# EternalEvan/InstaRevive

Hardware: AMD Instinct MI355X
Metric: 512->2048 one-step SR images/sec (higher is better)
Workload: dtype bf16; 1 GPU; 512x512 LQ, sr_scale 4 -> 2048x2048 network input, untiled, batch 1 per GPU, full SwinIR->VAE-enc->DiT(t=400)->VAE-dec path; global_batch=1, parallelism=dp1, weights=seeded random, full-size architectures

## Files before the change

### include/instarevive_hip.h

```cpp
#ifndef INSTAREVIVE_HIP_H
#define INSTAREVIVE_HIP_H
#include <stddef.h>
#include <stdint.h>
#ifdef __cplusplus
extern "C" {
#endif

typedef struct ir_ctx ir_ctx;

enum { IR_STAGE_SWINIR = 0, IR_STAGE_VAE_ENCODE = 1, IR_STAGE_DIT = 2, IR_STAGE_VAE_DECODE = 3, IR_STAGE_PIPELINE = 4,
       IR_STAGE_COLORFIX = 5, IR_STAGE_T5 = 6 ,
       IR_STAGE_CLDM = 7 , IR_STAGE_CLDM_PIPELINE = 8 ,
       IR_STAGE_CLIP_TEXT = 9 ,
       IR_STAGE_PNG = 10 ,
       IR_STAGE_RESAMPLE = 11 ,
       IR_STAGE_METRICS = 12 ,
       IR_STAGE_LPIPS = 13 ,
       IR_STAGE_NIQE = 14 ,
       IR_STAGE_CLIPIQA = 15 ,
       IR_STAGE_DEGRADE = 16  };
enum { IR_FLAG_NO_PREPROCESS = 1, IR_FLAG_TILED = 2, IR_FLAG_FIX_WAVELET = 4, IR_FLAG_FIX_ADAIN = 8,
       IR_FLAG_CONTROL_LQ = 16,
       IR_FLAG_GRAPH = 32,
       IR_FLAG_FP8 = 64 };
// ... 169 lines not shown
int ir_op_geglu(ir_ctx* ctx, void* stream, const uint16_t* ag, uint16_t* out, long rows, int f);

int ir_op_attention_d512_fp8(ir_ctx* ctx, void* stream, const uint16_t* q, const uint16_t* k, const uint16_t* v, uint16_t* o, int b, int t, float scale,
                             void* ws, size_t ws_bytes);
int ir_op_attention_fp8(ir_ctx* ctx, void* stream, const uint16_t* q, const uint16_t* k, const uint16_t* v, uint16_t* o, int b, int heads, int t,
                        float scale, void* ws, size_t ws_bytes);
int ir_op_swin_attention(ir_ctx* ctx, void* stream, const uint16_t* qkv, uint16_t* out, const float* bias_t, int b, int h, int w,
                         int heads, int shift, float scale);
int ir_op_swin_mlp(ir_ctx* ctx, void* stream, const float* x, float* out, uint16_t* out2, const void* w_tiles, const float* vec, long t, int c,
                   int hid_p, float eps, const float* next_g, const float* next_b, const void* qkv_tiles, const float* qkv_b, int qkv_n);
int ir_op_swin_attn_proj(ir_ctx* ctx, void* stream, const uint16_t* qkv, const float* xres, float* out, const void* proj_t, const float* proj_b,
                         const float* bias_t, int b, int h, int w, int shift, float scale);
int ir_op_swin_block(ir_ctx* ctx, void* stream, const uint16_t* qkv, const float* x_in, float* x_out, uint16_t* out2, const void* proj_t,
                     const float* proj_b, const float* bias_t, int b, int h, int w, int shift, float scale, const void* w_tiles, const float* vec,
                     int c, int hid_p, float eps, const float* next_g, const float* next_b, const void* qkv_tiles, const float* qkv_b, int qkv_n);
int ir_op_softmax_rows(ir_ctx* ctx, void* stream, const float* x, uint16_t* y, int rows, int cols);
int ir_op_nchw_to_nhwc(ir_ctx* ctx, void* stream, const float* in, uint16_t* out, int n, int ch, long hw, int cpad, float scale, float shift);
int ir_op_nhwc_to_nchw(ir_ctx* ctx, void* stream, const float* in, int in_cs, float* out, int n, int ch, long hw, float scale, float shift, int clamp01);

#ifdef __cplusplus
}
#endif
#endif
```

### instarevive_amd/_lib.py

```python
import ctypes as C
import os

import torch

_HERE = os.path.dirname(os.path.abspath(__file__))
LIB_PATH = os.environ.get("INSTAREVIVE_HIP_LIB") or os.path.join(_HERE, "csrc", "libinstarevive_hip.so")

SYMBOLS = [
    "ir_abi_version", "ir_init", "ir_destroy", "ir_last_error", "ir_upload", "ir_drop_optional", "ir_has_tensor",
    "ir_swinir_configure", "ir_vae_configure", "ir_dit_configure", "ir_dit_control_configure", "ir_dit_set_prompt", "ir_t5_configure", "ir_t5_encode", "ir_workspace_bytes",
    "ir_swinir_forward", "ir_vae_encode", "ir_dit_forward", "ir_dit_step", "ir_dit_forward_control", "ir_dit_step_control", "ir_vae_decode", "ir_color_fix",
    "ir_pipeline", "ir_u8_to_nchw", "ir_nchw_to_u8", "ir_profile_begin", "ir_profile_select", "ir_profile_end", "ir_profile_end_kernels", "ir_profile_kernel_count",
    "ir_profile_kernel_name",
    "ir_op_conv", "ir_op_conv_splitk", "ir_op_conv_groupnorm", "ir_op_linear", "ir_op_groupnorm", "ir_op_layernorm", "ir_op_attention", "ir_op_swin_attention",
    "ir_op_swin_mlp", "ir_op_swin_attn_proj", "ir_op_swin_block", "ir_op_dit_block", "ir_op_softmax_rows", "ir_op_nchw_to_nhwc", "ir_op_nhwc_to_nchw",
    "ir_tiled_count", "ir_tiled_encode", "ir_tiled_encode_part", "ir_tiled_encode_overflow", "ir_op_conv_up2x2", "ir_op_conv_norm", "ir_op_vae_conv_in", "ir_op_vae_norm_conv_out", "ir_op_conv64", "ir_op_conv64_to3", "ir_tiled_dit", "ir_tiled_blend_latent", "ir_tiled_decode", "ir_tiled_blend_pixels", "ir_set_plain_kernels", "ir_set_fp8", "ir_set_fp8_mask", "ir_attn_fallback_count", "ir_op_conv_fp8", "ir_op_conv_fp8_up", "ir_op_conv_fp8_route", "ir_fp8_features", "ir_op_attention_fp8", "ir_op_attention_d512_fp8",
    "ir_unet_configure", "ir_unet_set_context", "ir_cldm_sample", "ir_cldm_pipeline", "ir_clip_text_configure", "ir_clip_text_encode", "ir_op_groupnorm_any", "ir_op_geglu",
    "ir_dit_set_prompts", "ir_op_attention_kv_groups", "ir_graph_records", "ir_op_vae_segment", "ir_op_vae_segment_ws", "ir_op_vae_segment_info",
    "ir_png_bound", "ir_png_encode", "ir_resample_plan_bytes", "ir_resample_plan", "ir_resample_u8", "ir_metrics_y",
    "ir_lpips_scale_table", "ir_lpips_configure", "ir_lpips", "ir_niqe_window", "ir_niqe_stats",
    "ir_clipiqa_scale_table", "ir_clipiqa_configure", "ir_clipiqa", "ir_degrade_qtables", "ir_degrade",
]

STAGE_SWINIR, STAGE_VAE_ENCODE, STAGE_DIT, STAGE_VAE_DECODE, STAGE_PIPELINE, STAGE_COLORFIX, STAGE_T5, STAGE_CLDM, STAGE_CLDM_PIPELINE, STAGE_CLIP_TEXT, STAGE_PNG, STAGE_RESAMPLE, STAGE_METRICS = range(13)
STAGE_LPIPS = 13
STAGE_NIQE = 14
STAGE_CLIPIQA = 15
STAGE_DEGRADE = 16
DEGRADE_NORM_NONE, DEGRADE_NORM_MAX = 0, 1
DEGRADE_MAX_KSIZE, DEGRADE_MIN_LOW = 41, 8
# ... 62 lines not shown
    lib.ir_profile_kernel_name.argtypes = [i]
    lib.ir_profile_kernel_name.restype = C.c_char_p
    lib.ir_u8_to_nchw.argtypes = [vp, vp, vp, vp, i, i, i]
    lib.ir_nchw_to_u8.argtypes = [vp, vp, vp, vp, i, i, i]
    lib.ir_op_conv.argtypes = [vp, vp, vp, vp, vp, vp, i, i, i, i, i, i, i, i, i, i, i, f, vp, i, i]
    lib.ir_op_conv_splitk.argtypes = [vp, vp, vp, vp, vp, vp, i, i, i, i, i, i, i, vp, i, i, vp, sz, C.POINTER(C.c_int)]
    lib.ir_op_conv_groupnorm.argtypes = [vp, vp, vp, vp, vp, vp, vp, vp, vp, i, i, i, i, i, i, i, vp, i, vp, sz, C.POINTER(C.c_int)]
    lib.ir_op_linear.argtypes = [vp, vp, vp, vp, vp, vp, i, i, i, i, i, vp, vp, i, i, f]
    lib.ir_op_groupnorm.argtypes = [vp, vp, vp, vp, vp, vp, i, i, i, i, f, i, vp, sz]
    lib.ir_op_layernorm.argtypes = [vp, vp, vp, vp, vp, vp, i, i, i, i, f]
    lib.ir_op_attention.argtypes = [vp, vp, vp, vp, vp, vp, i, i, i, i, i, f, vp, vp, sz]
    lib.ir_op_swin_attention.argtypes = [vp, vp, vp, vp, vp, i, i, i, i, i, f]
    lib.ir_op_swin_mlp.argtypes = [vp, vp, vp, vp, vp, vp, vp, C.c_long, i, i, f, vp, vp, vp, vp, i]
    lib.ir_op_swin_attn_proj.argtypes = [vp, vp, vp, vp, vp, vp, vp, vp, i, i, i, i, f]
    lib.ir_op_swin_block.argtypes = [vp, vp, vp, vp, vp, vp, vp, vp, vp, i, i, i, i, f, vp, vp, i, i, f, vp, vp, vp, vp, i]
    lib.ir_op_dit_block.argtypes = [vp, vp, vp, i, i, i, i, f, vp, sz]
    lib.ir_op_softmax_rows.argtypes = [vp, vp, vp, vp, i, i]
    lib.ir_op_nchw_to_nhwc.argtypes = [vp, vp, vp, vp, i, i, C.c_long, i, f, f]
    lib.ir_op_nhwc_to_nchw.argtypes = [vp, vp, vp, i, vp, i, i, C.c_long, f, f, i]
    lib.ir_tiled_count.argtypes = [i, i, i, i]
    lib.ir_tiled_encode.argtypes = [vp, vp, vp, vp, vp, vp, i, i, i, i, f, vp, sz]
    lib.ir_tiled_encode_part.argtypes = [vp, vp, vp, vp, vp, vp, i, i, i, i, f, i, i, i, vp, vp, vp, sz]
    lib.ir_tiled_encode_overflow.argtypes = [vp, vp]
    lib.ir_op_conv_up2x2.argtypes = [vp, vp, vp, vp, vp, vp, i, i, i, i, i]
    lib.ir_op_conv_norm.argtypes = [vp, vp, vp, vp, vp, vp, vp, vp, vp, i, i, i, i, i]
    lib.ir_op_vae_conv_in.argtypes = [vp, vp, vp, vp, vp, vp, vp, i, i, i, f, f, vp]
    lib.ir_op_vae_norm_conv_out.argtypes = [vp, vp, vp, vp, vp, vp, vp, vp, i, i, i]
    lib.ir_op_conv64.argtypes = [vp, vp, vp, vp, vp, vp, i, i, i, i, f]
    lib.ir_op_conv64_to3.argtypes = [vp, vp, vp, vp, vp, vp, i, i, i]
    lib.ir_tiled_dit.argtypes = [vp, vp, vp, vp, i, i, i, i, i, i, i, f, f, i, vp, sz]
# ... 152 lines not shown
```

### instarevive_amd/csrc/api.cpp

```cpp
#include <hip/hip_runtime.h>
#include <math.h>
#include <stdarg.h>
#include <stdio.h>
#include <string.h>

#include <algorithm>
#include <memory>
#include <string>
#include <unordered_map>
#include <vector>

#include "../../include/instarevive_hip.h"
#include "kernels.h"

enum { ACT_NONE = 0, ACT_GELU_ERF = 1, ACT_GELU_TANH = 2, ACT_LRELU = 3, ACT_SILU = 4 };

namespace {

struct Tensor {
    void* p = nullptr;
    size_t bytes = 0;
};

struct Conv {
// ... 539 lines not shown
    float* xa = r.a.alloc<float>(T * Cp);
    float* xb = r.a.alloc<float>(T * Cp);
    bf16_t* xn = r.a.alloc<bf16_t>(T * Cp);
    bf16_t* qkv = r.a.alloc<bf16_t>(T * 3 * m.heads * 32);
    bf16_t* att = r.a.alloc<bf16_t>(T * Cp);
    bf16_t* hid = r.a.alloc<bf16_t>(T * m.hid_p);
    bf16_t* xc = r.a.alloc<bf16_t>(T * Cp);
    LAUNCH(r, PC_OTHER, 0.0, 0.0, ir_launch_swin_prep(in, f0, n, h, w, m.mean, m.range, r.s), "swin_prep");
    conv(r, m.conv_first, f0, n, gh, gw, 192, x0, Cp, 1, 1, 1, 0, ACT_NONE, 0.f, nullptr, 0, 0);
    layernorm(r, x0, nullptr, xa, m.pe.g, m.pe.b, T, m.C, Cp, Cp, 1e-5f);
    const float scale = 1.0f / sqrtf((float)m.C / (float)m.heads);
    for (const SwinLayer& L : m.layers) {
        const float* cur = xa;
        bool have_ln1 = false;
        bool have_qkv = false;
        for (size_t j = 0; j < L.blocks.size(); ++j) {
            const SwinBlock& b = L.blocks[j];
            const bool last = j + 1 == L.blocks.size();
            if (!have_qkv) {
                if (!have_ln1) layernorm(r, cur, xn, nullptr, b.n1.g, b.n1.b, T, m.C, Cp, Cp, 1e-5f);
                linear(r, b.qkv, xn, (int)T, Cp, qkv, 3 * m.heads * 32, 0, ACT_NONE, nullptr, 0, 0);
            }
            have_ln1 = have_qkv = false;
            const bool fuse_ln = !last && (m.C & 3) == 0;
            const SwinBlock* nb = fuse_ln ? &L.blocks[j + 1] : nullptr;
            const bool fuse_qkv = nb && nb->qkv_t && nb->qkv.b;
            const double f_attn = 4.0 * (double)T * 64 * m.C + 2.0 * (double)T * m.C * m.C;
            const double f_mlp = 4.0 * (double)T * m.C * m.hid + (fuse_qkv ? 6.0 * (double)T * m.C * m.C : 0.0);
            const double b_mlp = 4.0 * (double)T * m.C * 2 + (fuse_qkv ? 2.0 * (double)T * 3 * m.C : 0.0);
            bf16_t* mlp_out2 = last ? xc : (fuse_qkv ? qkv : (fuse_ln ? xn : nullptr));
            const int shift = (j & 1) ? 4 : 0;
            const float* fbias = shift ? b.biasM : b.biasT;
            const bool fused_attn = b.proj_t && fbias && !g_ir_plain_kernels && (long)T * 576 * 2 < (1L << 32);
            if (fused_attn && b.mlp_t) {
                LAUNCHK(r, PK_SWIN_BLOCK, f_attn + f_mlp, b_mlp + 2.0 * (double)T * 3 * m.C,
                       ir_launch_swin_block(qkv, cur, xb, mlp_out2, b.proj_t, b.proj.b, fbias, n, gh, gw, shift, scale, b.mlp_t, b.mlp_v, m.C, m.hid_p,
                                            1e-5f, r.s, nb ? nb->n1.g : nullptr, nb ? nb->n1.b : nullptr, fuse_qkv ? nb->qkv_t : nullptr,
                                            fuse_qkv ? nb->qkv.b : nullptr, fuse_qkv ? 3 * m.heads * 32 : 0), "swin_block");
                have_ln1 = fuse_ln && !fuse_qkv;
// ... 3164 lines not shown
}
int ir_op_swin_attn_proj(ir_ctx* c, void* stream, const uint16_t* qkv, const float* xres, float* out, const void* proj_t, const float* proj_b,
                         const float* bias_t, int b, int h, int w, int shift, float scale) {
    use_ctx(c);
    int rc = ir_launch_swin_attn_proj(qkv, xres, out, proj_t, proj_b, bias_t, b, h, w, shift, scale, (hipStream_t)stream);
    return rc ? fail(c, rc, "swin_attn_proj failed (%d)", rc) : 0;
}
int ir_op_swin_block(ir_ctx* c, void* stream, const uint16_t* qkv, const float* x_in, float* x_out, uint16_t* out2, const void* proj_t,
                     const float* proj_b, const float* bias_t, int b, int h, int w, int shift, float scale, const void* w_tiles, const float* vec,
                     int ch, int hid_p, float eps, const float* next_g, const float* next_b, const void* qkv_tiles, const float* qkv_b, int qkv_n) {
    use_ctx(c);
    int rc = ir_launch_swin_block(qkv, x_in, x_out, out2, proj_t, proj_b, bias_t, b, h, w, shift, scale, w_tiles, vec, ch, hid_p, eps,
                                  (hipStream_t)stream, next_g, next_b, qkv_tiles, qkv_b, qkv_n);
    return rc ? fail(c, rc, "swin_block failed (%d)", rc) : 0;
}
int ir_op_nchw_to_nhwc(ir_ctx* c, void* stream, const float* in, uint16_t* out, int n, int ch, long hw, int cpad, float scale, float shift) {
    use_ctx(c);
    int rc = ir_launch_nchw_to_nhwc_bf16(in, out, n, ch, hw, cpad, scale, shift, (hipStream_t)stream);
    return rc ? fail(c, rc, "nchw_to_nhwc failed (%d)", rc) : 0;
}
int ir_op_nhwc_to_nchw(ir_ctx* c, void* stream, const float* in, int in_cs, float* out, int n, int ch, long hw, float scale, float shift, int clamp01) {
    use_ctx(c);
    int rc = ir_launch_nhwc_to_nchw(in, in_cs, out, n, ch, hw, scale, shift, clamp01, (hipStream_t)stream);
    return rc ? fail(c, rc, "nhwc_to_nchw failed (%d)", rc) : 0;
}
int ir_op_groupnorm_any(ir_ctx* c, void* stream, const uint16_t* x, uint16_t* y, const float* gamma, const float* beta, int n, long hw, int ch,
                        int groups, float eps, int silu, void* ws, size_t ws_bytes) {
    if (!c || !x || !y || !ws) return fail(c, -1, "ir_op_groupnorm_any: null argument");
    if (ws_bytes < (size_t)ir_gn_any_ws_floats(n, hw, ch) * 4) return fail(c, -20, "ir_op_groupnorm_any: workspace too small");
    use_ctx(c);
// ... 17 lines not shown
```

### instarevive_amd/csrc/kernels.h

```cpp
#pragma once
#include <hip/hip_runtime.h>
#include <stdint.h>

typedef uint16_t bf16_t;

extern int g_ir_plain_kernels;

struct IGemmParams {
    const bf16_t* in;
    int NB, H, W;
    int Cin;
    int in_cs;
    int Ho, Wo;
    int taps;
    int stride;
    int pad;
    int up;
    const bf16_t* wgt;
    long wgt_rs;
    int Cout, Cout_pad, M;
    const float* bias;
    int act;
    float slope;
    float out_scale;
// ... 96 lines not shown
int ir_launch_swin_attn(const bf16_t* qkv, bf16_t* out, const float* biasT, int B, int H, int W, int heads, int ld, int ldo,
                        int shift, float scale, hipStream_t s);
int ir_launch_softmax_rows(const float* x, bf16_t* y, long rows, int cols, long ldx, long ldy, hipStream_t s);
static inline int ir_attn_dv(int D) { return (D + 31) & ~31; }

int ir_launch_swin_mlp(const float* x, float* out, bf16_t* out2, const void* w_tiles, const float* vec, long T, int C, int hid_p, float eps,
                       hipStream_t s, const float* next_g = nullptr, const float* next_b = nullptr, const void* qkv_tiles = nullptr,
                       const float* qkv_b = nullptr, int qkv_n = 0);
int ir_launch_swin_attn_proj(const bf16_t* qkv, const float* xres, float* out, const void* proj_t, const float* proj_b, const float* biasT, int B,
                             int H, int W, int shift, float scale, hipStream_t s);

int ir_launch_swin_block(const bf16_t* qkv, const float* x_in, float* x_out, bf16_t* out2, const void* proj_t, const float* proj_b, const float* biasT,
                         int B, int H, int W, int shift, float scale, const void* w_tiles, const float* vec, int C, int hid_p, float eps, hipStream_t s,
                         const float* next_g = nullptr, const float* next_b = nullptr, const void* qkv_tiles = nullptr, const float* qkv_b = nullptr,
                         int qkv_n = 0);

int ir_launch_t5_embed(const int* ids, const bf16_t* table, float* x, long rows, int D, int vocab, int* bad, hipStream_t s);
int ir_launch_t5_rmsnorm(const float* x, const float* w, bf16_t* yb, float* yf, long rows, int D, float eps, hipStream_t s);
int ir_launch_t5_attn(const bf16_t* qkv, const float* bias, const float* key_mask, bf16_t* out, int B, int T, int H, int dk, hipStream_t s);
int ir_launch_t5_gated_gelu(const bf16_t* ab, bf16_t* out, long rows, int F, hipStream_t s);

#ifndef IR_PNG_ROWS
#define IR_PNG_ROWS 8
#endif
#define IR_PNG_HEADER_BITS 1106
int ir_launch_png_encode(const uint8_t* img, int n, int h, long pitch, int vh, int vw, uint8_t* out, size_t out_stride, uint32_t* info,
                         uint32_t* hist, uint32_t* codes, uint32_t* header, uint32_t* chunk_bytes, uint8_t* slots, long slot_cap, hipStream_t s);

#define IR_RESAMPLE_MAGIC 0x52535038
#define IR_RESAMPLE_HEADER 16
// ... 107 lines not shown
```

### instarevive_amd/csrc/swin_fused.hip

```cpp
#include "common.h"
#include "kernels.h"

typedef __attribute__((address_space(3))) void* sw_lds_t;
IR_DEVINL void sw_glds16(const void* g, sw_lds_t l) { __builtin_amdgcn_global_load_lds(g, l, 16, 0, 0); }

namespace swf {
constexpr int CP = 192;
constexpr int W1_ROW = 400, W1_TILE = 13312;
constexpr int W2_ROW = 80, W2_TILE = 15360;
constexpr int SLOT = W1_TILE + W2_TILE;
constexpr int PIECES = SLOT / 1024;
constexpr int VEC_OFF = 2 * SLOT;
constexpr int NEXT_OFF = 1152;
constexpr int STG_OFF = VEC_OFF + 6144;
constexpr int STG_WAVE = 3 * 4096;
constexpr int LDS_TOTAL = STG_OFF + 8 * STG_WAVE;
}

template <bool LN_NEXT, bool QKV = false>
__global__ __launch_bounds__(512, 1) void swin_mlp_kernel(const float* __restrict__ x, float* __restrict__ out, bf16_t* __restrict__ out2,
                                                          const unsigned char* __restrict__ w, const float* __restrict__ vec, long T, int C,
                                                          int NJ, float eps, const float* __restrict__ next_g, const float* __restrict__ next_b,
                                                          const unsigned char* __restrict__ wq, const float* __restrict__ bq, int NQ) {
    using namespace swf;
// ... 415 lines not shown
    }
}

int ir_launch_swin_attn_proj(const bf16_t* qkv, const float* xres, float* out, const void* proj_t, const float* proj_b, const float* biasT, int B,
                             int H, int W, int shift, float scale, hipStream_t s) {
    if (H <= 0 || W <= 0 || (H & 7) || (W & 7) || shift < 0 || shift >= 8 || B <= 0) return -2;
    if ((long)B * H * W * 576 * 2 >= (1L << 32)) return -4;
    const long n_waves = 2L * B * (H >> 3) * (W >> 3);
    const long blocks = (n_waves + 3) / 4;
    if (blocks > 0x7fffffffL) return -4;
    hipLaunchKernelGGL(swin_attn_proj_kernel, dim3((unsigned)blocks), dim3(256), 0, s, qkv, xres, out, reinterpret_cast<const bf16_t*>(proj_t), proj_b, biasT, H, W,
                       shift, scale * 1.44269504088896340736f, n_waves);
    return hipGetLastError() == hipSuccess ? 0 : -1;
}

template <bool LN_NEXT, bool QKV>
__global__ __launch_bounds__(512, 1) void swin_block_kernel(const bf16_t* __restrict__ qkv, const float* __restrict__ x_in, float* __restrict__ x_out,
                                                            bf16_t* __restrict__ out2, const bf16_t* __restrict__ proj_t,
                                                            const float* __restrict__ proj_b, const float* __restrict__ biasT, int H, int W, int shift,
                                                            float scale_log2, long n_waves, const unsigned char* __restrict__ w,
                                                            const float* __restrict__ vec, int C, int NJ, float eps, const float* __restrict__ next_g,
                                                            const float* __restrict__ next_b, const unsigned char* __restrict__ wq,
                                                            const float* __restrict__ bq, int NQ) {
    using namespace swf;
    constexpr int HEADS = 6, LD = 3 * CP;
#ifdef IR_SWIN_STAMPS
    unsigned long long stp[8];
    stp[0] = __builtin_amdgcn_s_memrealtime();
#define IR_STAMP(k) stp[k] = __builtin_amdgcn_s_memrealtime()
#else
#define IR_STAMP(k)
#endif
    extern __shared__ __attribute__((aligned(1024))) unsigned char smem[];
    const int tid = threadIdx.x, lane = tid & 63, wid = tid >> 6;
    const int wu = __builtin_amdgcn_readfirstlane(wid);
    const int r = lane & 31, h = lane >> 5;
    long wv = (long)blockIdx.x * 8 + wu;
    const bool active = wv < n_waves;
    if (!active) wv = n_waves - 1;

    const int NS = NJ + (QKV ? NQ / 2 : 0);
    auto stage = [&](int jt, int slot) {
        const unsigned char* src = (QKV && jt >= NJ ? wq + (long)(jt - NJ) * SLOT : w + (long)jt * SLOT) + lane * 16;
#pragma unroll
        for (int i = 0; i < 4; ++i)
            if (wu + 8 * i < PIECES) sw_glds16(src + (wu + 8 * i) * 1024, (sw_lds_t)(smem + slot * SLOT + (wu + 8 * i) * 1024));
    };
    stage(0, 0);
    float* vs = reinterpret_cast<float*>(smem + VEC_OFF);
    const int nvec = 3 * CP + 32 * NJ;
    for (int i = tid; i < nvec; i += 512) vs[i] = vec[i];
    constexpr bool ln_next = LN_NEXT;
    if (ln_next)
        for (int i = tid; i < 2 * CP; i += 512) {
            const int c = i < CP ? i : i - CP;
            vs[NEXT_OFF + i] = c < C ? (i < CP ? next_g[c] : next_b[c]) : 0.f;
        }

    const int g = (int)(wv & 1);
    long wlin = wv >> 1;
    const int nwx = W >> 3, nwy = H >> 3;
    const int wx = (int)(wlin % nwx); wlin /= nwx;
    const int wy = (int)(wlin % nwy);
    const long img = wlin / nwy;
    auto tok = [&](int i) {
        int y = wy * 8 + (i >> 3) + shift, x = wx * 8 + (i & 7) + shift;
        if (y >= H) y -= H;
        if (x >= W) x -= W;
        return (long)y * W + x;
    };
    const long tbase = img * H * W;
    const long qtok = tbase + tok(32 * g + r);
    f32x16 yacc[6];
    {
        const long ktok[2] = {tbase + tok(r), tbase + tok(32 + r)};
        const int cls = shift ? ((wy == nwy - 1 ? 2 : 0) | (wx == nwx - 1 ? 1 : 0)) : 0;
        bf16x8 idf[2];
#pragma unroll
        for (int ks = 0; ks < 2; ++ks) {
            uint32_t w4[4];
#pragma unroll
            for (int e2 = 0; e2 < 4; ++e2) {
                const int c0 = 16 * ks + 8 * h + 2 * e2;
                w4[e2] = (c0 == r ? 0x3f80u : 0u) | (c0 + 1 == r ? 0x3f800000u : 0u);
            }
            idf[ks] = __builtin_bit_cast(bf16x8, make_uint4(w4[0], w4[1], w4[2], w4[3]));
        }
#pragma unroll
        for (int ct = 0; ct < 6; ++ct)
// ... 61 lines not shown
                    o = mfma32(__builtin_bit_cast(bf16x8, swa_pack8(vt, 8 * s2, 1.0f)), __builtin_bit_cast(bf16x8, swa_pack8_valu(s[kt], 8 * s2, 1.0f)), o);
            }
            const float inv = 1.0f / rs;
            const bf16x8 ob[2] = {__builtin_bit_cast(bf16x8, swa_pack8_valu(o, 0, inv)), __builtin_bit_cast(bf16x8, swa_pack8_valu(o, 8, inv))};
#pragma unroll
            for (int ct = 0; ct < 6; ++ct)
#pragma unroll
                for (int s2 = 0; s2 < 2; ++s2) {
                    const bf16x8 wp = *reinterpret_cast<const bf16x8*>(proj_t + (((hd * 6 + ct) * 2 + s2) * 64 + lane) * 8);
                    yacc[ct] = mfma32(wp, ob[s2], yacc[ct]);
                }
        }
    }

    IR_STAMP(1);
    unsigned char* stg = smem + STG_OFF + wu * STG_WAVE;
    const int ptok = lane >> 3, pslot = lane & 7;
    long gtk[4];
#pragma unroll
    for (int pc = 0; pc < 4; ++pc) gtk[pc] = tbase + tok(32 * g + 8 * pc + ptok);
    auto load_half = [&](int t0) {
#pragma unroll
        for (int ts = 0; ts < 3; ++ts)
#pragma unroll
            for (int pc = 0; pc < 4; ++pc) {
                const int tk = 8 * pc + ptok;
                sw_glds16(x_in + gtk[pc] * CP + 32 * (t0 + ts) + 4 * (pslot ^ ((tk >> 1) & 7)), (sw_lds_t)(stg + ts * 4096 + pc * 1024));
            }
    };
    auto frag_addr = [&](int ts, int i) { return stg + ts * 4096 + r * 128 + (((2 * i + h) ^ ((r >> 1) & 7)) << 4); };
    f32x4 xr[6][4];
#pragma unroll
    for (int hf = 0; hf < 2; ++hf) {
        load_half(3 * hf);
        wait_dma();
#pragma unroll
        for (int ts = 0; ts < 3; ++ts)
#pragma unroll
            for (int i = 0; i < 4; ++i) {
                const int t = 3 * hf + ts;
                const f32x4 pb = *reinterpret_cast<const f32x4*>(proj_b + 32 * t + 8 * i + 4 * h);
                xr[t][i] = f32x4{yacc[t][4 * i], yacc[t][4 * i + 1], yacc[t][4 * i + 2], yacc[t][4 * i + 3]} + pb + *reinterpret_cast<const f32x4*>(frag_addr(ts, i));
            }
        __builtin_amdgcn_fence(__ATOMIC_RELEASE, "wavefront");
        asm volatile("s_waitcnt lgkmcnt(0)" ::: "memory");
// ... 35 lines not shown
    }
    f32x16 y[6];
#pragma unroll
    for (int ot = 0; ot < 6; ++ot)
#pragma unroll
        for (int i = 0; i < 4; ++i) {
            const f32x4 b2 = *reinterpret_cast<const f32x4*>(vs + 2 * CP + 32 * NJ + 32 * ot + 8 * i + 4 * h);
#pragma unroll
            for (int e = 0; e < 4; ++e) y[ot][4 * i + e] = xr[ot][i][e] + b2[e];
        }
    const int a1 = r * W1_ROW + h * 16;
    const int a2 = W1_TILE + r * W2_ROW + h * 16;
    for (int jt = 0; jt < NJ; ++jt) {
        wait_dma();
        __syncthreads();
        if (jt + 1 < NS) stage(jt + 1, (jt + 1) & 1);
        const unsigned char* sl = smem + (jt & 1) * SLOT;
        f32x16 hacc;
#pragma unroll
        for (int e = 0; e < 16; ++e) hacc[e] = 0.f;
#pragma unroll
        for (int s = 0; s < 12; ++s) hacc = mfma32(*reinterpret_cast<const bf16x8*>(sl + a1 + s * 32), xn[s], hacc);
        bf16x8 hb[2];
#pragma unroll
        for (int q = 0; q < 2; ++q) {
            uint32_t wv4[4];
#pragma unroll
            for (int u = 0; u < 2; ++u) {
                const f32x4 b1 = *reinterpret_cast<const f32x4*>(vs + 2 * CP + 32 * jt + 16 * q + 8 * u + 4 * h);
                const int g0 = 8 * q + 4 * u;
                wv4[2 * u] = pack2bf(gelu_erf(hacc[g0] + b1[0]), gelu_erf(hacc[g0 + 1] + b1[1]));
                wv4[2 * u + 1] = pack2bf(gelu_erf(hacc[g0 + 2] + b1[2]), gelu_erf(hacc[g0 + 3] + b1[3]));
            }
            hb[q] = __builtin_bit_cast(bf16x8, make_uint4(wv4[0], wv4[1], wv4[2], wv4[3]));
        }
#pragma unroll
        for (int ot = 0; ot < 6; ++ot)
#pragma unroll
            for (int q = 0; q < 2; ++q) y[ot] = mfma32(*reinterpret_cast<const bf16x8*>(sl + a2 + ot * 32 * W2_ROW + q * 32), hb[q], y[ot]);
    }
    IR_STAMP(3);
#pragma unroll
    for (int hf = 0; hf < 2; ++hf) {
#pragma unroll
        for (int ts = 0; ts < 3; ++ts)
#pragma unroll
            for (int i = 0; i < 4; ++i) {
                const int t = 3 * hf + ts;
                const f32x4 nx = f32x4{y[t][4 * i], y[t][4 * i + 1], y[t][4 * i + 2], y[t][4 * i + 3]};
                *reinterpret_cast<f32x4*>(frag_addr(ts, i)) = nx;
                if (ln_next) xr[t][i] = nx;
            }
        __builtin_amdgcn_fence(__ATOMIC_RELEASE, "wavefront");
        asm volatile("s_waitcnt lgkmcnt(0)" ::: "memory");
        __builtin_amdgcn_wave_barrier();
#pragma unroll
// ... 122 lines not shown
    const unsigned char* wq = reinterpret_cast<const unsigned char*>(qkv_tiles);
    auto go = [&](auto kern) {
        static bool attr_set = false;
        if (!attr_set) {
            if (hipFuncSetAttribute(reinterpret_cast<const void*>(kern), hipFuncAttributeMaxDynamicSharedMemorySize, (int)lds) != hipSuccess) return -1;
            attr_set = true;
        }
        hipLaunchKernelGGL(kern, dim3((unsigned)blocks), dim3(512), lds, s, qkv, x_in, x_out, out2, pt, proj_b, biasT, H, W, shift, sl2, n_waves, wt, vec, C, NJ, eps,
                           next_g, next_b, wq, qkv_b, NQ);
        return hipGetLastError() == hipSuccess ? 0 : -1;
    };
    if (qkv_tiles) return go(swin_block_kernel<true, true>);
    if (next_g) return go(swin_block_kernel<true, false>);
    return go(swin_block_kernel<false, false>);
}
```

Before: 8.471 images/sec.

## Fuse LayerNorm and QKV projection into the head of the Swin block kernel

```diff
diff --git a/include/instarevive_hip.h b/include/instarevive_hip.h
--- a/include/instarevive_hip.h
+++ b/include/instarevive_hip.h
@@ -207,6 +207,9 @@
 int ir_op_swin_block(ir_ctx* ctx, void* stream, const uint16_t* qkv, const float* x_in, float* x_out, uint16_t* out2, const void* proj_t,
                      const float* proj_b, const float* bias_t, int b, int h, int w, int shift, float scale, const void* w_tiles, const float* vec,
                      int c, int hid_p, float eps, const float* next_g, const float* next_b, const void* qkv_tiles, const float* qkv_b, int qkv_n);
+int ir_op_swin_block_hq(ir_ctx* ctx, void* stream, const float* n1_g, const float* n1_b, const void* qkv_tiles, const float* qkv_b, int qkv_n,
+                        const float* x_in, float* x_out, uint16_t* out2, const void* proj_t, const float* proj_b, const float* bias_t, int b, int h,
+                        int w, int shift, float scale, const void* w_tiles, const float* vec, int c, int hid_p, float eps);
 int ir_op_softmax_rows(ir_ctx* ctx, void* stream, const float* x, uint16_t* y, int rows, int cols);
 int ir_op_nchw_to_nhwc(ir_ctx* ctx, void* stream, const float* in, uint16_t* out, int n, int ch, long hw, int cpad, float scale, float shift);
 int ir_op_nhwc_to_nchw(ir_ctx* ctx, void* stream, const float* in, int in_cs, float* out, int n, int ch, long hw, float scale, float shift, int clamp01);
diff --git a/instarevive_amd/_lib.py b/instarevive_amd/_lib.py
--- a/instarevive_amd/_lib.py
+++ b/instarevive_amd/_lib.py
@@ -13,7 +13,7 @@
     "ir_pipeline", "ir_u8_to_nchw", "ir_nchw_to_u8", "ir_profile_begin", "ir_profile_select", "ir_profile_end", "ir_profile_end_kernels", "ir_profile_kernel_count",
     "ir_profile_kernel_name",
     "ir_op_conv", "ir_op_conv_splitk", "ir_op_conv_groupnorm", "ir_op_linear", "ir_op_groupnorm", "ir_op_layernorm", "ir_op_attention", "ir_op_swin_attention",
-    "ir_op_swin_mlp", "ir_op_swin_attn_proj", "ir_op_swin_block", "ir_op_dit_block", "ir_op_softmax_rows", "ir_op_nchw_to_nhwc", "ir_op_nhwc_to_nchw",
+    "ir_op_swin_mlp", "ir_op_swin_attn_proj", "ir_op_swin_block", "ir_op_swin_block_hq", "ir_op_dit_block", "ir_op_softmax_rows", "ir_op_nchw_to_nhwc", "ir_op_nhwc_to_nchw",
     "ir_tiled_count", "ir_tiled_encode", "ir_tiled_encode_part", "ir_tiled_encode_overflow", "ir_op_conv_up2x2", "ir_op_conv_norm", "ir_op_vae_conv_in", "ir_op_vae_norm_conv_out", "ir_op_conv64", "ir_op_conv64_to3", "ir_tiled_dit", "ir_tiled_blend_latent", "ir_tiled_decode", "ir_tiled_blend_pixels", "ir_set_plain_kernels", "ir_set_fp8", "ir_set_fp8_mask", "ir_attn_fallback_count", "ir_op_conv_fp8", "ir_op_conv_fp8_up", "ir_op_conv_fp8_route", "ir_fp8_features", "ir_op_attention_fp8", "ir_op_attention_d512_fp8",
     "ir_unet_configure", "ir_unet_set_context", "ir_cldm_sample", "ir_cldm_pipeline", "ir_clip_text_configure", "ir_clip_text_encode", "ir_op_groupnorm_any", "ir_op_geglu",
     "ir_dit_set_prompts", "ir_op_attention_kv_groups", "ir_graph_records", "ir_op_vae_segment", "ir_op_vae_segment_ws", "ir_op_vae_segment_info",
@@ -106,6 +106,7 @@
     lib.ir_op_swin_mlp.argtypes = [vp, vp, vp, vp, vp, vp, vp, C.c_long, i, i, f, vp, vp, vp, vp, i]
     lib.ir_op_swin_attn_proj.argtypes = [vp, vp, vp, vp, vp, vp, vp, vp, i, i, i, i, f]
     lib.ir_op_swin_block.argtypes = [vp, vp, vp, vp, vp, vp, vp, vp, vp, i, i, i, i, f, vp, vp, i, i, f, vp, vp, vp, vp, i]
+    lib.ir_op_swin_block_hq.argtypes = [vp, vp, vp, vp, vp, vp, i, vp, vp, vp, vp, vp, vp, i, i, i, i, f, vp, vp, i, i, f]
     lib.ir_op_dit_block.argtypes = [vp, vp, vp, i, i, i, i, f, vp, sz]
     lib.ir_op_softmax_rows.argtypes = [vp, vp, vp, vp, i, i]
     lib.ir_op_nchw_to_nhwc.argtypes = [vp, vp, vp, vp, i, i, C.c_long, i, f, f]
diff --git a/instarevive_amd/csrc/api.cpp b/instarevive_amd/csrc/api.cpp
--- a/instarevive_amd/csrc/api.cpp
+++ b/instarevive_amd/csrc/api.cpp
@@ -577,15 +577,30 @@
         const float* cur = xa;
         bool have_ln1 = false;
         bool have_qkv = false;
+        auto head_qkv = [&](size_t k) {
+            const SwinBlock& bk = L.blocks[k];
+            return k > 0 && bk.qkv_t && bk.qkv.b && bk.proj_t && ((k & 1) ? bk.biasM : bk.biasT) && bk.mlp_t && !g_ir_plain_kernels && (m.C & 3) == 0 &&
+                   m.heads == 6 && Cp == 192 && (long)T * 576 * 2 < (1L << 32);
+        };
         for (size_t j = 0; j < L.blocks.size(); ++j) {
             const SwinBlock& b = L.blocks[j];
             const bool last = j + 1 == L.blocks.size();
+            if (head_qkv(j)) {
+                const int sh = (j & 1) ? 4 : 0;
+                LAUNCHK(r, PK_SWIN_BLOCK, 4.0 * (double)T * 64 * m.C + 2.0 * (double)T * m.C * m.C + 4.0 * (double)T * m.C * m.hid + 6.0 * (double)T * m.C * m.C,
+                       4.0 * (double)T * m.C * 2,
+                       ir_launch_swin_block_hq(b.n1.g, b.n1.b, b.qkv_t, b.qkv.b, 3 * m.heads * 32, cur, xb, last ? xc : nullptr, b.proj_t, b.proj.b,
+                                               sh ? b.biasM : b.biasT, n, gh, gw, sh, scale, b.mlp_t, b.mlp_v, m.C, m.hid_p, 1e-5f, r.s), "swin_block_hq");
+                have_ln1 = have_qkv = false;
+                cur = xb;
+                continue;
+            }
             if (!have_qkv) {
                 if (!have_ln1) layernorm(r, cur, xn, nullptr, b.n1.g, b.n1.b, T, m.C, Cp, Cp, 1e-5f);
                 linear(r, b.qkv, xn, (int)T, Cp, qkv, 3 * m.heads * 32, 0, ACT_NONE, nullptr, 0, 0);
             }
             have_ln1 = have_qkv = false;
-            const bool fuse_ln = !last && (m.C & 3) == 0;
+            const bool fuse_ln = !last && (m.C & 3) == 0 && !head_qkv(j + 1);
             const SwinBlock* nb = fuse_ln ? &L.blocks[j + 1] : nullptr;
             const bool fuse_qkv = nb && nb->qkv_t && nb->qkv.b;
             const double f_attn = 4.0 * (double)T * 64 * m.C + 2.0 * (double)T * m.C * m.C;
@@ -3780,6 +3795,14 @@
                                   (hipStream_t)stream, next_g, next_b, qkv_tiles, qkv_b, qkv_n);
     return rc ? fail(c, rc, "swin_block failed (%d)", rc) : 0;
 }
+int ir_op_swin_block_hq(ir_ctx* c, void* stream, const float* n1_g, const float* n1_b, const void* qkv_tiles, const float* qkv_b, int qkv_n,
+                        const float* x_in, float* x_out, uint16_t* out2, const void* proj_t, const float* proj_b, const float* bias_t, int b, int h,
+                        int w, int shift, float scale, const void* w_tiles, const float* vec, int ch, int hid_p, float eps) {
+    use_ctx(c);
+    int rc = ir_launch_swin_block_hq(n1_g, n1_b, qkv_tiles, qkv_b, qkv_n, x_in, x_out, out2, proj_t, proj_b, bias_t, b, h, w, shift, scale, w_tiles, vec,
+                                     ch, hid_p, eps, (hipStream_t)stream);
+    return rc ? fail(c, rc, "swin_block_hq failed (%d)", rc) : 0;
+}
 int ir_op_nchw_to_nhwc(ir_ctx* c, void* stream, const float* in, uint16_t* out, int n, int ch, long hw, int cpad, float scale, float shift) {
     use_ctx(c);
     int rc = ir_launch_nchw_to_nhwc_bf16(in, out, n, ch, hw, cpad, scale, shift, (hipStream_t)stream);
diff --git a/instarevive_amd/csrc/kernels.h b/instarevive_amd/csrc/kernels.h
--- a/instarevive_amd/csrc/kernels.h
+++ b/instarevive_amd/csrc/kernels.h
@@ -134,6 +134,9 @@
                          int B, int H, int W, int shift, float scale, const void* w_tiles, const float* vec, int C, int hid_p, float eps, hipStream_t s,
                          const float* next_g = nullptr, const float* next_b = nullptr, const void* qkv_tiles = nullptr, const float* qkv_b = nullptr,
                          int qkv_n = 0);
+int ir_launch_swin_block_hq(const float* n1_g, const float* n1_b, const void* qkv_tiles, const float* qkv_b, int qkv_n, const float* x_in, float* x_out,
+                            bf16_t* out2, const void* proj_t, const float* proj_b, const float* biasT, int B, int H, int W, int shift, float scale,
+                            const void* w_tiles, const float* vec, int C, int hid_p, float eps, hipStream_t s);
 
 int ir_launch_t5_embed(const int* ids, const bf16_t* table, float* x, long rows, int D, int vocab, int* bad, hipStream_t s);
 int ir_launch_t5_rmsnorm(const float* x, const float* w, bf16_t* yb, float* yf, long rows, int D, float eps, hipStream_t s);
diff --git a/instarevive_amd/csrc/swin_fused.hip b/instarevive_amd/csrc/swin_fused.hip
--- a/instarevive_amd/csrc/swin_fused.hip
+++ b/instarevive_amd/csrc/swin_fused.hip
@@ -453,7 +453,7 @@
     return hipGetLastError() == hipSuccess ? 0 : -1;
 }
 
-template <bool LN_NEXT, bool QKV>
+template <bool LN_NEXT, bool QKV, bool HEAD_QKV = false>
 __global__ __launch_bounds__(512, 1) void swin_block_kernel(const bf16_t* __restrict__ qkv, const float* __restrict__ x_in, float* __restrict__ x_out,
                                                             bf16_t* __restrict__ out2, const bf16_t* __restrict__ proj_t,
                                                             const float* __restrict__ proj_b, const float* __restrict__ biasT, int H, int W, int shift,
@@ -471,26 +471,30 @@
 #define IR_STAMP(k)
 #endif
     extern __shared__ __attribute__((aligned(1024))) unsigned char smem[];
-    const int tid = threadIdx.x, lane = tid & 63, wid = tid >> 6;
+    const int tid = threadIdx.x, wid = tid >> 6;
     const int wu = __builtin_amdgcn_readfirstlane(wid);
-    const int r = lane & 31, h = lane >> 5;
+    int lane = tid & 63, r = lane & 31, h = lane >> 5;
     long wv = (long)blockIdx.x * 8 + wu;
     const bool active = wv < n_waves;
-    if (!active) wv = n_waves - 1;
+    static_assert(!HEAD_QKV || (!LN_NEXT && !QKV), "a block that computes its own q | k | v has the plain tail");
+    if (!active) wv = HEAD_QKV ? n_waves - 2 + (wu & 1) : n_waves - 1;
 
     const int NS = NJ + (QKV ? NQ / 2 : 0);
-    auto stage = [&](int jt, int slot) {
-        const unsigned char* src = (QKV && jt >= NJ ? wq + (long)(jt - NJ) * SLOT : w + (long)jt * SLOT) + lane * 16;
+    constexpr int R0 = HEAD_QKV ? 1 : 0;
+    auto stage_src = [&](const unsigned char* base, int slot) {
+        const unsigned char* src = base + lane * 16;
 #pragma unroll
         for (int i = 0; i < 4; ++i)
             if (wu + 8 * i < PIECES) sw_glds16(src + (wu + 8 * i) * 1024, (sw_lds_t)(smem + slot * SLOT + (wu + 8 * i) * 1024));
     };
-    stage(0, 0);
+    auto stage = [&](int jt, int slot) { stage_src(QKV && jt >= NJ ? wq + (long)(jt - NJ) * SLOT : w + (long)jt * SLOT, slot); };
+    if constexpr (HEAD_QKV) stage_src(wq, 0);
+    else stage(0, 0);
     float* vs = reinterpret_cast<float*>(smem + VEC_OFF);
     const int nvec = 3 * CP + 32 * NJ;
     for (int i = tid; i < nvec; i += 512) vs[i] = vec[i];
     constexpr bool ln_next = LN_NEXT;
-    if (ln_next)
+    if (ln_next || HEAD_QKV)
         for (int i = tid; i < 2 * CP; i += 512) {
             const int c = i < CP ? i : i - CP;
             vs[NEXT_OFF + i] = c < C ? (i < CP ? next_g[c] : next_b[c]) : 0.f;
@@ -510,8 +514,220 @@
     };
     const long tbase = img * H * W;
     const long qtok = tbase + tok(32 * g + r);
+    unsigned char* stg = smem + STG_OFF + wu * STG_WAVE;
+    int ptok = lane >> 3, pslot = lane & 7;
+    long gtk[4];
+    auto load_half = [&](int t0) {
+#pragma unroll
+        for (int ts = 0; ts < 3; ++ts)
+#pragma unroll
+            for (int pc = 0; pc < 4; ++pc) {
+                const int tk = 8 * pc + ptok;
+                sw_glds16(x_in + gtk[pc] * CP + 32 * (t0 + ts) + 4 * (pslot ^ ((tk >> 1) & 7)), (sw_lds_t)(stg + ts * 4096 + pc * 1024));
+            }
+    };
+    auto frag_addr = [&](int ts, int i) { return stg + ts * 4096 + r * 128 + (((2 * i + h) ^ ((r >> 1) & 7)) << 4); };
     f32x16 yacc[6];
-    {
+    if constexpr (HEAD_QKV) {
+#pragma unroll
+        for (int pc = 0; pc < 4; ++pc) gtk[pc] = tbase + tok(32 * g + 8 * pc + ptok);
+        bf16x8 xq[12];
+        {
+            f32x4 xr[6][4];
+#pragma unroll
+            for (int hf = 0; hf < 2; ++hf) {
+                load_half(3 * hf);
+                wait_dma();
+#pragma unroll
+                for (int ts = 0; ts < 3; ++ts)
+#pragma unroll
+                    for (int i = 0; i < 4; ++i) xr[3 * hf + ts][i] = *reinterpret_cast<const f32x4*>(frag_addr(ts, i));
+                __builtin_amdgcn_fence(__ATOMIC_RELEASE, "wavefront");
+                asm volatile("s_waitcnt lgkmcnt(0)" ::: "memory");
+            }
+            float t1 = 0.f;
+#pragma unroll
+            for (int t = 0; t < 6; ++t)
+#pragma unroll
+                for (int i = 0; i < 4; ++i) t1 += (xr[t][i][0] + xr[t][i][1]) + (xr[t][i][2] + xr[t][i][3]);
+            t1 += __shfl_xor(t1, 32);
+            float mean1 = t1 / (float)C;
+            float t2 = 0.f;
+#pragma unroll
+            for (int t = 0; t < 6; ++t)
+#pragma unroll
+                for (int i = 0; i < 4; ++i)
+#pragma unroll
+                    for (int e = 0; e < 4; ++e) {
+                        const float d = xr[t][i][e] - mean1;
+                        t2 += (32 * t + 8 * i + 4 * h + e < C) ? d * d : 0.f;
+                    }
+            t2 += __shfl_xor(t2, 32);
+            const float rstd1 = rsqrtf(t2 / (float)C + eps);
+            asm volatile("" : "+v"(mean1));
+            __syncthreads();
+#pragma unroll
+            for (int s = 0; s < 12; ++s) {
+                uint32_t wv4[4];
+#pragma unroll
+                for (int q = 0; q < 2; ++q) {
+                    const int t = s >> 1, i = 2 * (s & 1) + q, c0 = 32 * t + 8 * i + 4 * h;
+                    const f32x4 gg = *reinterpret_cast<const f32x4*>(vs + NEXT_OFF + c0), bb = *reinterpret_cast<const f32x4*>(vs + NEXT_OFF + CP + c0);
+                    const f32x4 v = (xr[t][i] - mean1) * rstd1 * gg + bb;
+                    wv4[2 * q] = pack2bf(v[0], v[1]);
+                    wv4[2 * q + 1] = pack2bf(v[2], v[3]);
+                }
+                asm volatile("" : "+v"(wv4[3]) : : "memory");
+                xq[s] = __builtin_bit_cast(bf16x8, make_uint4(wv4[0], wv4[1], wv4[2], wv4[3]));
+            }
+        }
+        int lq = lane;
+        asm volatile("" : "+v"(lq));
+        const int rq = lq & 31, hq = lq >> 5;
+        const int cls = shift ? ((wy == nwy - 1 ? 2 : 0) | (wx == nwx - 1 ? 1 : 0)) : 0;
+        bf16x8 idf[2];
+#pragma unroll
+        for (int ks = 0; ks < 2; ++ks) {
+            uint32_t w4[4];
+#pragma unroll
+            for (int e2 = 0; e2 < 4; ++e2) {
+                const int c0 = 16 * ks + 8 * hq + 2 * e2;
+                w4[e2] = (c0 == rq ? 0x3f80u : 0u) | (c0 + 1 == rq ? 0x3f800000u : 0u);
+            }
+            idf[ks] = __builtin_bit_cast(bf16x8, make_uint4(w4[0], w4[1], w4[2], w4[3]));
+        }
+        const float* brow = biasT + (long)cls * HEADS * 4096 + 32 * g + rq;
+        const int a1 = rq * W1_ROW + hq * 16;
+        const unsigned char* pair = smem + STG_OFF + (wu & ~1) * STG_WAVE + rq * 128;
+        const int sw = (rq >> 1) & 7;
+        bf16x8 obq[3][2][2];
+#pragma unroll
+        for (int a = 0; a < 3; ++a)
+#pragma unroll
+            for (int b = 0; b < 4; ++b) obq[a][b >> 1][b & 1] = __builtin_bit_cast(bf16x8, make_uint4(0u, 0u, 0u, 0u));
+#pragma unroll 1
+        for (int p = 0; p < 3; ++p) {
+#pragma unroll
+            for (int j = 0; j < 3; ++j) {
+                const int st = 3 * j + p;
+                f32x4 bv[2][4];
+#pragma unroll
+                for (int u = 0; u < 2; ++u)
+#pragma unroll
+                    for (int i = 0; i < 4; ++i) bv[u][i] = *reinterpret_cast<const f32x4*>(bq + 32 * (2 * st + u) + 8 * i + 4 * hq);
+                wait_dma();
+                __syncthreads();
+                stage_src(j < 2 ? wq + (long)(st + 3) * SLOT : (p < 2 ? wq + (long)(p + 1) * SLOT : w), (p + j + 1) & 1);
+                const unsigned char* sl = smem + ((p + j) & 1) * SLOT;
+                unsigned char* sb = stg + j * 4096;
+#pragma unroll
+                for (int u = 0; u < 2; ++u) {
+                    f32x16 acc;
+#pragma unroll
+                    for (int e = 0; e < 16; ++e) acc[e] = 0.f;
+#pragma unroll
+                    for (int s = 0; s < 12; ++s) acc = mfma32(*reinterpret_cast<const bf16x8*>(sl + u * W1_TILE + a1 + s * 32), xq[s], acc);
+#pragma unroll
+                    for (int i = 0; i < 4; ++i)
+                        *reinterpret_cast<uint2*>(sb + rq * 128 + (((4 * u + i) ^ sw) << 4) + 8 * hq) =
+                            make_uint2(pack2bf(acc[4 * i] + bv[u][i][0], acc[4 * i + 1] + bv[u][i][1]), pack2bf(acc[4 * i + 2] + bv[u][i][2], acc[4 * i + 3] + bv[u][i][3]));
+                }
+            }
+            __syncthreads();
+#pragma unroll
+            for (int b = 0; b < 4; ++b) {
+                obq[0][b >> 1][b & 1] = obq[1][b >> 1][b & 1];
+                obq[1][b >> 1][b & 1] = obq[2][b >> 1][b & 1];
+            }
+#pragma unroll
+            for (int hh = 0; hh < 2; ++hh) {
+                const int hd = 2 * p + hh;
+                bf16x8 qf[2], kf[2][2], vf[2][2];
+#pragma unroll
+                for (int ks = 0; ks < 2; ++ks) {
+                    const int po = ((4 * hh + 2 * ks + hq) ^ sw) << 4;
+                    qf[ks] = *reinterpret_cast<const bf16x8*>(stg + rq * 128 + po);
+#pragma unroll
+                    for (int kt = 0; kt < 2; ++kt) {
+                        kf[kt][ks] = *reinterpret_cast<const bf16x8*>(pair + kt * STG_WAVE + 4096 + po);
+                        vf[kt][ks] = *reinterpret_cast<const bf16x8*>(pair + kt * STG_WAVE + 8192 + po);
+                    }
+                }
+                f32x16 s[2];
+#pragma unroll
+                for (int kt = 0; kt < 2; ++kt) {
+#pragma unroll
+                    for (int e = 0; e < 16; ++e) s[kt][e] = 0.f;
+#pragma unroll
+                    for (int ks = 0; ks < 2; ++ks) s[kt] = mfma32(kf[kt][ks], qf[ks], s[kt]);
+                }
+                const float* bt = brow + (long)hd * 4096;
+                float mx = -INFINITY;
+#pragma unroll
+                for (int kt = 0; kt < 2; ++kt)
+#pragma unroll
+                    for (int e = 0; e < 16; ++e) {
+                        const int key = 32 * kt + (e & 3) + 8 * (e >> 2) + 4 * hq;
+                        const float v = s[kt][e] * scale_log2 + bt[key * 64];
+                        s[kt][e] = v;
+                        mx = fmaxf(mx, v);
+                    }
+                mx = xhalf_max(mx);
+                float rs = 0.f;
+#pragma unroll
+                for (int kt = 0; kt < 2; ++kt)
+#pragma unroll
+                    for (int e = 0; e < 16; ++e) {
+                        const float pv = __builtin_amdgcn_exp2f(s[kt][e] - mx);
+                        s[kt][e] = pv;
+                        rs += pv;
+                    }
+                rs += __shfl_xor(rs, 32);
+                f32x16 o;
+#pragma unroll
+                for (int e = 0; e < 16; ++e) o[e] = 0.f;
+#pragma unroll
+                for (int kt = 0; kt < 2; ++kt) {
+                    f32x16 vt;
+#pragma unroll
+                    for (int e = 0; e < 16; ++e) vt[e] = 0.f;
+#pragma unroll
+                    for (int ks = 0; ks < 2; ++ks) vt = mfma32(vf[kt][ks], idf[ks], vt);
+#pragma unroll
+                    for (int s2 = 0; s2 < 2; ++s2)
+                        o = mfma32(__builtin_bit_cast(bf16x8, swa_pack8(vt, 8 * s2, 1.0f)), __builtin_bit_cast(bf16x8, swa_pack8_valu(s[kt], 8 * s2, 1.0f)), o);
+                }
+                const float inv = 1.0f / rs;
+                obq[2][hh][0] = __builtin_bit_cast(bf16x8, swa_pack8_valu(o, 0, inv));
+                obq[2][hh][1] = __builtin_bit_cast(bf16x8, swa_pack8_valu(o, 8, inv));
+            }
+        }
+        __syncthreads();
+        lane = lq;
+        asm volatile("" : "+v"(lane));
+        r = lane & 31, h = lane >> 5, ptok = lane >> 3, pslot = lane & 7;
+#pragma unroll
+        for (int ct = 0; ct < 6; ++ct)
+#pragma unroll
+            for (int e = 0; e < 16; ++e) yacc[ct][e] = 0.f;
+        bf16x8 wp[2][6];
+        auto load_wp = [&](int gi) {
+#pragma unroll
+            for (int c = 0; c < 6; ++c) wp[gi & 1][c] = *reinterpret_cast<const bf16x8*>(proj_t + ((gi * 6 + c) * 64 + lane) * 8);
+        };
+        load_wp(0);
+#pragma unroll
+        for (int gi = 0; gi < 12; ++gi) {
+            if (gi + 1 < 12) load_wp(gi + 1);
+            asm volatile("" ::: "memory");
+#pragma unroll
+            for (int c = 0; c < 6; ++c) {
+                const int hd = gi >> 1, ct = 3 * (gi & 1) + (c >> 1);
+                yacc[ct] = mfma32(wp[gi & 1][c], obq[hd >> 1][hd & 1][c & 1], yacc[ct]);
+            }
+        }
+        __builtin_amdgcn_sched_barrier(0);
+    } else {
         const long ktok[2] = {tbase + tok(r), tbase + tok(32 + r)};
         const int cls = shift ? ((wy == nwy - 1 ? 2 : 0) | (wx == nwx - 1 ? 1 : 0)) : 0;
         bf16x8 idf[2];
@@ -603,21 +819,8 @@
     }
 
     IR_STAMP(1);
-    unsigned char* stg = smem + STG_OFF + wu * STG_WAVE;
-    const int ptok = lane >> 3, pslot = lane & 7;
-    long gtk[4];
 #pragma unroll
     for (int pc = 0; pc < 4; ++pc) gtk[pc] = tbase + tok(32 * g + 8 * pc + ptok);
-    auto load_half = [&](int t0) {
-#pragma unroll
-        for (int ts = 0; ts < 3; ++ts)
-#pragma unroll
-            for (int pc = 0; pc < 4; ++pc) {
-                const int tk = 8 * pc + ptok;
-                sw_glds16(x_in + gtk[pc] * CP + 32 * (t0 + ts) + 4 * (pslot ^ ((tk >> 1) & 7)), (sw_lds_t)(stg + ts * 4096 + pc * 1024));
-            }
-    };
-    auto frag_addr = [&](int ts, int i) { return stg + ts * 4096 + r * 128 + (((2 * i + h) ^ ((r >> 1) & 7)) << 4); };
     f32x4 xr[6][4];
 #pragma unroll
     for (int hf = 0; hf < 2; ++hf) {
@@ -683,8 +886,8 @@
     for (int jt = 0; jt < NJ; ++jt) {
         wait_dma();
         __syncthreads();
-        if (jt + 1 < NS) stage(jt + 1, (jt + 1) & 1);
-        const unsigned char* sl = smem + (jt & 1) * SLOT;
+        if (jt + 1 < NS) stage(jt + 1, (jt + 1 + R0) & 1);
+        const unsigned char* sl = smem + ((jt + R0) & 1) * SLOT;
         f32x16 hacc;
 #pragma unroll
         for (int e = 0; e < 16; ++e) hacc[e] = 0.f;
@@ -709,6 +912,12 @@
             for (int q = 0; q < 2; ++q) y[ot] = mfma32(*reinterpret_cast<const bf16x8*>(sl + a2 + ot * 32 * W2_ROW + q * 32), hb[q], y[ot]);
     }
     IR_STAMP(3);
+    if constexpr (HEAD_QKV) {
+        asm volatile("" : "+v"(lane));
+        r = lane & 31, h = lane >> 5, ptok = lane >> 3, pslot = lane & 7;
+#pragma unroll
+        for (int pc = 0; pc < 4; ++pc) gtk[pc] = tbase + tok(32 * g + 8 * pc + ptok);
+    }
 #pragma unroll
     for (int hf = 0; hf < 2; ++hf) {
 #pragma unroll
@@ -861,3 +1070,24 @@
     if (next_g) return go(swin_block_kernel<true, false>);
     return go(swin_block_kernel<false, false>);
 }
+
+int ir_launch_swin_block_hq(const float* n1_g, const float* n1_b, const void* qkv_tiles, const float* qkv_b, int qkv_n, const float* x_in, float* x_out,
+                            bf16_t* out2, const void* proj_t, const float* proj_b, const float* biasT, int B, int H, int W, int shift, float scale,
+                            const void* w_tiles, const float* vec, int C, int hid_p, float eps, hipStream_t s) {
+    if (H <= 0 || W <= 0 || (H & 7) || (W & 7) || shift < 0 || shift >= 8 || B <= 0) return -2;
+    if (C <= 0 || C > swf::CP || (C & 3) || hid_p <= 0 || (hid_p & 31) || hid_p > 512) return -2;
+    if (!n1_g || !n1_b || !qkv_tiles || !qkv_b || qkv_n != 576) return -2;
+    const long n_waves = 2L * B * (H >> 3) * (W >> 3);
+    const long blocks = (n_waves + 7) / 8;
+    if (blocks > 0x7fffffffL) return -4;
+    const size_t lds = swf::LDS_TOTAL;
+    static bool attr_set = false;
+    if (!attr_set) {
+        if (hipFuncSetAttribute(reinterpret_cast<const void*>(swin_block_kernel<false, false, true>), hipFuncAttributeMaxDynamicSharedMemorySize, (int)lds) != hipSuccess) return -1;
+        attr_set = true;
+    }
+    hipLaunchKernelGGL((swin_block_kernel<false, false, true>), dim3((unsigned)blocks), dim3(512), lds, s, (const bf16_t*)nullptr, x_in, x_out, out2,
+                       reinterpret_cast<const bf16_t*>(proj_t), proj_b, biasT, H, W, shift, scale * 1.44269504088896340736f, n_waves,
+                       reinterpret_cast<const unsigned char*>(w_tiles), vec, C, hid_p / 32, eps, n1_g, n1_b, reinterpret_cast<const unsigned char*>(qkv_tiles), qkv_b, 18);
+    return hipGetLastError() == hipSuccess ? 0 : -1;
+}
```

After: 8.460 images/sec. No clear change (-0.1%).
